# stevewongv/Sparse2Dense

Hardware: AMD Instinct MI355X
Metric: LiDAR frames/sec (fwd+bwd), 150k-pt 0.1m-voxel synthetic Waymo scene (higher is better)
Workload: dtype bf16 (sparse stack: bf16 storage; dense neck/head: bf16 NHWC activations; fp32 accumulate, statistics, master weights, optimizer)

## Files before the change

### include/s2d_debug.h

```cpp
#ifndef S2D_DEBUG_H
#define S2D_DEBUG_H

#include "s2d.h"

#ifdef __cplusplus
extern "C" {
#endif

int s2d_debug_lds_fill(float value, int blocks, int spin, float *sink, s2d_stream_t stream);

void s2d_debug_rg_trace(void *buf);

int s2d_conv2d_debug_force(int bm, int ns, int shared_a, int conv1x1_k64);

int s2d_conv2d_plan(int kind, int n, int h, int w, int cin, int cout, int pad, int stride, int ks, int32_t out[8]);

int s2d_conv2d_wgrad_debug_force(int ring_deep, int splits);

int s2d_conv2d_wgrad_plan(int kind, int n, int h, int w, int c_in_role, int c_out_role, int pad, int ks, int32_t out[8]);

#ifdef __cplusplus
}
#endif

#endif
```

### sparse2dense_amd/_lib.py

```python
import ctypes
import os

_HERE = os.path.dirname(os.path.abspath(__file__))
LIB_PATH = os.path.join(_HERE, "lib", "libs2d_hip.so")

c_i32p = ctypes.c_void_p
c_f32p = ctypes.c_void_p
_I3 = ctypes.c_int32 * 3
_PFN_GEO = [ctypes.c_int64, ctypes.c_int, ctypes.c_int, ctypes.c_float, ctypes.c_float, ctypes.c_float, ctypes.c_float]
_F3 = ctypes.c_float * 3
_F6 = ctypes.c_float * 6


class CenterTask(ctypes.Structure):
    _fields_ = [(n, ctypes.c_void_p) for n in ("hm_logit", "reg", "height", "dim", "vel", "rot", "hm", "ind", "mask", "cat", "anno_box", "p",
                                               "d_logit", "d_reg", "d_height", "d_dim", "d_vel", "d_rot")] + [("classes", ctypes.c_int)]

class CenterPredictTask(ctypes.Structure):
    _fields_ = [("map", ctypes.c_void_p * 6), ("channel_stride", ctypes.c_int64 * 6), ("pixel_stride", ctypes.c_int64 * 6),
                ("classes", ctypes.c_int), ("label_base", ctypes.c_int)]


class AnchorPredictTask(ctypes.Structure):
    _fields_ = [(n, ctypes.c_void_p) for n in ("box_preds", "cls_preds", "dir_cls_preds", "anchors")] + \
# ... 233 lines not shown
    "s2d_bev_iou_f32": (ctypes.c_int, [c_f32p, ctypes.c_int, c_f32p, ctypes.c_int, c_f32p, ctypes.c_void_p]),
    "s2d_nms_workspace_bytes": (ctypes.c_size_t, [ctypes.c_int]),
    "s2d_nms_rotated_bev": (ctypes.c_int, [c_f32p, ctypes.c_int, ctypes.c_float, ctypes.c_int, ctypes.c_void_p, ctypes.c_void_p, ctypes.c_void_p,
                                           ctypes.c_size_t, ctypes.c_void_p]),
    "s2d_nms_circle": (ctypes.c_int, [c_f32p, ctypes.c_int, ctypes.c_float, ctypes.c_int, ctypes.c_void_p, ctypes.c_void_p, ctypes.c_void_p,
                                      ctypes.c_size_t, ctypes.c_void_p]),
    "s2d_center_predict_score": (ctypes.c_int, [ctypes.c_void_p] + [ctypes.c_int] * 5 + [ctypes.c_float, ctypes.c_void_p] + [ctypes.c_float] * 5 +
                                 [ctypes.c_void_p] * 4),
    "s2d_center_predict_boxes": (ctypes.c_int, [ctypes.c_void_p] + [ctypes.c_int] * 5 + [ctypes.c_float] * 5 + [ctypes.c_void_p] * 5 +
                                 [ctypes.c_int, ctypes.c_int64] + [ctypes.c_void_p] * 4),
    "s2d_nms_batched_workspace_bytes": (ctypes.c_size_t, [ctypes.c_int64, ctypes.c_int]),
    "s2d_nms_rotated_bev_batched": (ctypes.c_int, [c_f32p, ctypes.c_int, c_i32p, c_i32p, ctypes.c_int, ctypes.c_int, ctypes.c_int64, ctypes.c_float,
                                                   ctypes.c_int, ctypes.c_void_p, ctypes.c_void_p, ctypes.c_void_p, ctypes.c_size_t, ctypes.c_void_p]),
    "s2d_nms_circle_batched": (ctypes.c_int, [c_f32p, ctypes.c_int, c_i32p, c_i32p, ctypes.c_int, ctypes.c_int, ctypes.c_int64, c_f32p,
                                              ctypes.c_int, ctypes.c_void_p, ctypes.c_void_p, ctypes.c_void_p, ctypes.c_size_t, ctypes.c_void_p]),
    "s2d_segment_topk": (ctypes.c_int, [ctypes.c_void_p, ctypes.c_int, ctypes.c_int64, ctypes.c_int64, ctypes.c_int, ctypes.c_void_p, ctypes.c_void_p,
                                        ctypes.c_void_p, ctypes.c_int64] + [ctypes.c_void_p] * 4),
    "s2d_predict_static_gather": (ctypes.c_int, [ctypes.c_void_p] * 6 + [ctypes.c_int] * 4 + [ctypes.c_int64] + [ctypes.c_void_p] * 5),
    "s2d_assign_label": (ctypes.c_int, [c_f32p, c_i32p, ctypes.c_int, ctypes.c_int, ctypes.c_float * 2, ctypes.c_float * 2] + [ctypes.c_int] * 5 +
                         [ctypes.c_double, ctypes.c_int] + [ctypes.c_void_p] * 7),
    "s2d_assign_label_tasks": (ctypes.c_int, [c_f32p, c_i32p, ctypes.c_int, ctypes.c_int, ctypes.POINTER(ctypes.c_int32), ctypes.c_int,
                                              ctypes.c_float * 2, ctypes.c_float * 2] + [ctypes.c_int] * 4 + [ctypes.c_double, ctypes.c_int] +
                               [ctypes.c_void_p] * 7),
    "s2d_adam_max_tensors": (ctypes.c_int, []),
    "s2d_adam_step_f32": (ctypes.c_int, [ctypes.c_int] + [ctypes.c_void_p] * 5 + [ctypes.c_float] * 5 + [ctypes.c_int, c_f32p, ctypes.c_void_p]),
    "s2d_grad_norm_workspace_floats": (ctypes.c_size_t, [ctypes.c_int, ctypes.c_void_p]),
    "s2d_grad_sumsq_f32": (ctypes.c_int, [ctypes.c_int, ctypes.c_void_p, ctypes.c_void_p, c_f32p, ctypes.c_void_p, ctypes.c_void_p]),
    "s2d_grad_norm_finalize_f32": (ctypes.c_int, [c_f32p, ctypes.c_int, ctypes.c_float, c_f32p, ctypes.c_void_p]),
    "s2d_dwconv7_supported": (ctypes.c_int, [ctypes.c_int]),
    "s2d_dwconv7_nhwc_bf16": (ctypes.c_int, [ctypes.c_void_p, c_f32p, c_f32p] + [ctypes.c_int] * 5 + [ctypes.c_void_p, ctypes.c_void_p]),
    "s2d_dwconv7_wgrad_workspace_bytes": (ctypes.c_size_t, [ctypes.c_int] * 4),
    "s2d_dwconv7_wgrad_nhwc_bf16": (ctypes.c_int, [ctypes.c_void_p, ctypes.c_void_p] + [ctypes.c_int] * 4 +
                                    [c_f32p, c_f32p, ctypes.c_void_p, ctypes.c_size_t, ctypes.c_void_p]),
    "s2d_comm_allreduce_sum_f32": (ctypes.c_int, [ctypes.c_void_p, ctypes.c_int64, ctypes.c_void_p]),
    "s2d_conv2d3x3_supported": (ctypes.c_int, [ctypes.c_int, ctypes.c_int]),
    "s2d_conv2d3x3_stats_tiles": (ctypes.c_int64, [ctypes.c_int] * 7),
    "s2d_conv2d3x3_pack_weights_bf16": (ctypes.c_int, [c_f32p, ctypes.c_int, ctypes.c_int, ctypes.c_int, ctypes.c_int,
                                                       ctypes.c_void_p, ctypes.c_void_p]),
    "s2d_conv2d3x3_tile_rows": (ctypes.c_int, [ctypes.c_int] * 7),
    "s2d_conv2d3x3_nhwc_bf16": (ctypes.c_int, [ctypes.c_void_p, ctypes.c_void_p, c_f32p, ctypes.c_void_p] +
                                [ctypes.c_int] * 7 + [ctypes.c_void_p, c_f32p, ctypes.c_void_p]),
    "s2d_bn_partials_finalize_f32": (ctypes.c_int, [c_f32p, ctypes.c_int, ctypes.c_int64, ctypes.c_int, c_f32p, c_f32p,
                                                    ctypes.c_float, ctypes.c_float, c_f32p, c_f32p, c_f32p, c_f32p, c_f32p, c_f32p,
                                                    ctypes.c_void_p, ctypes.c_void_p]),
    "s2d_bn_partials_finalize_ws_f32": (ctypes.c_int, [c_f32p, ctypes.c_int, ctypes.c_int64, ctypes.c_int, c_f32p, c_f32p,
                                                       ctypes.c_float, ctypes.c_float, c_f32p, c_f32p, c_f32p, c_f32p, c_f32p, c_f32p,
                                                       ctypes.c_void_p, ctypes.c_void_p, ctypes.c_size_t, ctypes.c_void_p]),
    "s2d_conv2d3x3_bnbwd_supported": (ctypes.c_int, [ctypes.c_int] * 4),
    "s2d_conv2d3x3_nhwc_bf16_bnbwd": (ctypes.c_int, [ctypes.c_void_p] * 3 + [ctypes.c_int] * 6 + [ctypes.c_void_p, ctypes.c_void_p, c_f32p, c_f32p,
                                                                                                    ctypes.c_int, c_f32p, ctypes.c_void_p]),
    "s2d_conv2d_debug_force": (ctypes.c_int, [ctypes.c_int] * 4),
    "s2d_conv2d_plan": (ctypes.c_int, [ctypes.c_int] * 9 + [ctypes.POINTER(ctypes.c_int32)]),
    "s2d_conv2d_wgrad_debug_force": (ctypes.c_int, [ctypes.c_int] * 2),
    "s2d_conv2d_wgrad_plan": (ctypes.c_int, [ctypes.c_int] * 8 + [ctypes.POINTER(ctypes.c_int32)]),
    "s2d_conv2d1x1_bnbwd_supported": (ctypes.c_int, [ctypes.c_int] * 2),
    "s2d_conv2d1x1_nhwc_bf16_bnbwd": (ctypes.c_int, [ctypes.c_void_p] * 3 + [ctypes.c_int] * 5 + [ctypes.c_void_p, ctypes.c_void_p, c_f32p, c_f32p,
                                                                                                    ctypes.c_int, c_f32p, ctypes.c_void_p]),
    "s2d_bn_partials_bwd_finalize_ws_f32": (ctypes.c_int, [c_f32p, ctypes.c_int, ctypes.c_int64, ctypes.c_int, c_f32p, c_f32p, c_f32p, c_f32p,
                                                           c_f32p, c_f32p, c_f32p, c_f32p, ctypes.c_void_p, ctypes.c_size_t, ctypes.c_void_p]),
    "s2d_bn_partials_sum_f32": (ctypes.c_int, [c_f32p, ctypes.c_int, ctypes.c_int64, ctypes.c_int, c_f32p, ctypes.c_int,
                                               ctypes.c_void_p]),
    "s2d_bn_partials_sum_workspace_bytes": (ctypes.c_size_t, [ctypes.c_int, ctypes.c_int]),
    "s2d_bn_partials_sum_ws_f32": (ctypes.c_int, [c_f32p, ctypes.c_int, ctypes.c_int64, ctypes.c_int, c_f32p, ctypes.c_int,
                                                  ctypes.c_void_p, ctypes.c_size_t, ctypes.c_void_p]),
    "s2d_bnrow_workspace_bytes": (ctypes.c_size_t, [ctypes.c_int64, ctypes.c_int]),
    "s2d_bnrow_stats_bf16": (ctypes.c_int, [ctypes.c_void_p, ctypes.c_int64, ctypes.c_int, c_f32p, ctypes.c_int, ctypes.c_void_p, ctypes.c_size_t, ctypes.c_void_p]),
    "s2d_bnrow_stats_finalize_bf16": (ctypes.c_int, [ctypes.c_void_p, ctypes.c_int64, ctypes.c_int, c_f32p, c_f32p, ctypes.c_float, ctypes.c_float, c_f32p, c_f32p, c_f32p, c_f32p, c_f32p, c_f32p, ctypes.c_void_p, ctypes.c_void_p, ctypes.c_size_t, ctypes.c_void_p]),
    "s2d_bnrow_apply_bf16": (ctypes.c_int, [ctypes.c_void_p, c_f32p, c_f32p, ctypes.c_void_p, ctypes.c_int, ctypes.c_int64, ctypes.c_int, ctypes.c_void_p, ctypes.c_void_p]),
    "s2d_bnrow_bwd_reduce_bf16": (ctypes.c_int, [ctypes.c_void_p, ctypes.c_void_p, ctypes.c_void_p, c_f32p, c_f32p, ctypes.c_int, ctypes.c_int64, ctypes.c_int, c_f32p, c_f32p, ctypes.c_void_p, ctypes.c_size_t, ctypes.c_void_p]),
    "s2d_bnrow_bwd_reduce_finalize_bf16": (ctypes.c_int, [ctypes.c_void_p, ctypes.c_void_p, ctypes.c_void_p, c_f32p, c_f32p, ctypes.c_int, ctypes.c_int64, ctypes.c_int, c_f32p, c_f32p, c_f32p, c_f32p, c_f32p, c_f32p, c_f32p, c_f32p, ctypes.c_void_p, ctypes.c_size_t, ctypes.c_void_p]),
    "s2d_bnrow_bwd_apply_bf16": (ctypes.c_int, [ctypes.c_void_p, ctypes.c_void_p, ctypes.c_void_p, c_f32p, c_f32p, ctypes.c_int, c_f32p, c_f32p, c_f32p, ctypes.c_int64, ctypes.c_int, ctypes.c_void_p, ctypes.c_void_p, ctypes.c_void_p]),
    "s2d_bnrow_apply_ld_bf16": (ctypes.c_int, [ctypes.c_void_p, c_f32p, c_f32p, ctypes.c_void_p, ctypes.c_int, ctypes.c_int64, ctypes.c_int, ctypes.c_void_p,
                                               ctypes.c_int, ctypes.c_void_p]),
    "s2d_bnrow_bwd_reduce_ld_bf16": (ctypes.c_int, [ctypes.c_void_p, ctypes.c_int, ctypes.c_void_p, ctypes.c_void_p, c_f32p, c_f32p, ctypes.c_int, ctypes.c_int64,
                                                    ctypes.c_int, c_f32p, c_f32p, ctypes.c_void_p, ctypes.c_size_t, ctypes.c_void_p]),
    "s2d_bnrow_bwd_reduce_finalize_ld_bf16": (ctypes.c_int, [ctypes.c_void_p, ctypes.c_int, ctypes.c_void_p, ctypes.c_void_p, c_f32p, c_f32p, ctypes.c_int,
                                                             ctypes.c_int64, ctypes.c_int, c_f32p, c_f32p, c_f32p, c_f32p, c_f32p, c_f32p, c_f32p, c_f32p,
                                                             ctypes.c_void_p, ctypes.c_size_t, ctypes.c_void_p]),
    "s2d_bnrow_bwd_apply_ld_bf16": (ctypes.c_int, [ctypes.c_void_p, ctypes.c_int, ctypes.c_void_p, ctypes.c_void_p, c_f32p, c_f32p, ctypes.c_int, c_f32p, c_f32p,
                                                   c_f32p, ctypes.c_int64, ctypes.c_int, ctypes.c_void_p, ctypes.c_void_p, ctypes.c_void_p]),
    "s2d_upsample2x_nhwc_bf16": (ctypes.c_int, [ctypes.c_void_p] + [ctypes.c_int] * 4 + [ctypes.c_void_p, ctypes.c_void_p]),
    "s2d_upsample2x_bwd_nhwc_bf16": (ctypes.c_int, [ctypes.c_void_p] + [ctypes.c_int] * 4 + [ctypes.c_void_p, ctypes.c_void_p]),
    "s2d_maxpool2x2_nhwc_bf16": (ctypes.c_int, [ctypes.c_void_p] + [ctypes.c_int] * 4 + [ctypes.c_void_p, ctypes.c_void_p]),
    "s2d_maxpool2x2_bwd_nhwc_bf16": (ctypes.c_int, [ctypes.c_void_p, ctypes.c_void_p] + [ctypes.c_int] * 4 + [ctypes.c_void_p, ctypes.c_void_p]),
    "s2d_spconv_s16_supported": (ctypes.c_int, [ctypes.c_int, ctypes.c_int]),
    "s2d_debug_rg_trace": (None, [ctypes.c_void_p]),
    "s2d_spconv_s16_packed_elems": (ctypes.c_size_t, [ctypes.c_int, ctypes.c_int, ctypes.c_int]),
    "s2d_spconv_s16_pack_weights": (ctypes.c_int, [c_f32p, ctypes.c_int, ctypes.c_int, ctypes.c_int, ctypes.c_int, ctypes.c_int,
                                                   ctypes.c_int64, ctypes.c_void_p, ctypes.c_void_p]),
    "s2d_spconv_s16_pack_weights_pair": (ctypes.c_int, [c_f32p, ctypes.c_int, ctypes.c_int, ctypes.c_int, ctypes.c_int, ctypes.c_int64,
                                                        ctypes.c_int64, ctypes.c_void_p, ctypes.c_void_p, ctypes.c_void_p]),
    "s2d_spconv_s16_fwd": (ctypes.c_int, [ctypes.c_void_p, ctypes.c_int64, ctypes.c_void_p, c_f32p, c_i32p, ctypes.c_int64,
                                          ctypes.c_int, ctypes.c_int, ctypes.c_int, ctypes.c_void_p, ctypes.c_void_p,
                                          ctypes.c_void_p]),
    "s2d_spconv_s16_stats_tiles": (ctypes.c_int64, [ctypes.c_int64, ctypes.c_int, ctypes.c_int, ctypes.c_int]),
    "s2d_spconv_s16_fwd_stats": (ctypes.c_int, [ctypes.c_void_p, ctypes.c_int64, ctypes.c_void_p, c_f32p, c_i32p, ctypes.c_int64,
                                                ctypes.c_int, ctypes.c_int, ctypes.c_int, ctypes.c_void_p, ctypes.c_void_p, c_f32p,
                                                ctypes.c_void_p]),
    "s2d_rulebook_sort_workspace_bytes": (ctypes.c_size_t, [ctypes.c_int64]),
    "s2d_rulebook_sort_chunk_rows": (ctypes.c_int64, [ctypes.c_int64]),
    "s2d_rulebook_sort_by_mask": (ctypes.c_int, [c_i32p, ctypes.c_int, ctypes.c_int64, c_i32p, ctypes.c_void_p, c_i32p, ctypes.c_void_p, ctypes.c_size_t,
                                                 ctypes.c_void_p]),
    "s2d_spconv_s16_set_sorted_rows": (ctypes.c_int, [ctypes.c_int]),
    "s2d_spconv_s16_sorted_supported": (ctypes.c_int, [ctypes.c_int] * 3),
    "s2d_spconv_s16_fwd_sorted": (ctypes.c_int, [ctypes.c_void_p, ctypes.c_int64, ctypes.c_void_p, c_f32p, c_i32p, c_i32p, ctypes.c_void_p, ctypes.c_int64,
                                                 ctypes.c_int, ctypes.c_int, ctypes.c_int, ctypes.c_void_p, c_f32p, ctypes.c_void_p]),
# ... 208 lines not shown
```

### sparse2dense_amd/csrc/convt3d_mfma.hip

```cpp
#include "s2d_common.h"
#include <algorithm>
#include <cstdlib>

namespace s2d {

typedef float f32x4m __attribute__((ext_vector_type(4)));
typedef __bf16 bf16x8m __attribute__((ext_vector_type(8)));

constexpr unsigned CT_OOB = BUF_OOB;
__device__ __forceinline__ __amdgpu_buffer_rsrc_t ct_rsrc(const void *base, unsigned bytes) { return buf_rsrc(base, bytes); }
__device__ __forceinline__ f32x4m ct_load4(__amdgpu_buffer_rsrc_t r, unsigned voff, unsigned soff) { return buf_load4(r, voff, soff); }
typedef uint32_t u32x2m __attribute__((ext_vector_type(2)));
typedef uint32_t u32x3m __attribute__((ext_vector_type(3)));
typedef uint32_t u32x4m __attribute__((ext_vector_type(4)));
__device__ __forceinline__ u32x3m ct_load3u(__amdgpu_buffer_rsrc_t r, unsigned voff, unsigned soff) {
    return __builtin_bit_cast(u32x3m, __builtin_amdgcn_raw_buffer_load_b96(r, voff, soff, 0));
}
__device__ __forceinline__ u32x4m ct_load4u(__amdgpu_buffer_rsrc_t r, unsigned voff, unsigned soff) {
    return __builtin_bit_cast(u32x4m, __builtin_amdgcn_raw_buffer_load_b128(r, voff, soff, 0));
}
__device__ __forceinline__ u32x2m ct_load2u(__amdgpu_buffer_rsrc_t r, unsigned voff, unsigned soff) {
    return __builtin_bit_cast(u32x2m, __builtin_amdgcn_raw_buffer_load_b64(r, voff, soff, 0));
}
__device__ __forceinline__ uint32_t ct_hi_hi(uint32_t a, uint32_t b) { return __builtin_amdgcn_perm(b, a, 0x07060302u); }
// ... 833 lines not shown
                f32x4m v0[MT], v1[MT];
#pragma unroll
                for (int mt = 0; mt < MT; ++mt) {
                    v0[mt] = ct_load4(dr, (pos[mt] | pl0) >= CT_OOB ? CT_OOB : pos[mt] + pl0, soff);
                    v1[mt] = ct_load4(dr, (pos[mt] | pl1) >= CT_OOB ? CT_OOB : pos[mt] + pl1, soff);
                }
#pragma unroll
                for (int mt = 0; mt < MT; ++mt) {
                    bf16x8m a;
#pragma unroll
                    for (int e = 0; e < 4; ++e) {
                        float s0 = shifted[mt] ? (e ? v0[mt][e - (e ? 1 : 0)] : 0.f) : v0[mt][e];
                        float s1 = shifted[mt] ? (e ? v1[mt][e - (e ? 1 : 0)] : 0.f) : v1[mt][e];
                        if (e == 3) {
                            s0 = last[mt] ? 0.f : s0;
                            s1 = last[mt] ? 0.f : s1;
                        }
                        a[e] = (__bf16)s0;
                        a[4 + e] = (__bf16)s1;
                    }
#pragma unroll
                    for (int nt = 0; nt < NT; ++nt) acc[mt][nt] = __builtin_amdgcn_mfma_f32_16x16x32_bf16(a, bfr[nt], acc[mt][nt], 0, 0, 0);
                }
                }
            }
        }
        const __amdgpu_buffer_rsrc_t ir = ct_rsrc(din + (int64_t)n * s.cin * cells, ibytes);
        const unsigned rowoff = (unsigned)(((int64_t)hz * s.h + hy) * s.w * IS);
#pragma unroll
        for (int mt = 0; mt < MT; ++mt) {
            const int c0 = x0 + mt * 16 + 4 * q;
#pragma unroll
            for (int nt = 0; nt < NT; ++nt) {
                const int ci = nt * 16 + r;
                const unsigned plane = ci < s.cin ? (unsigned)(ci * cells * IS) : CT_OOB;
                if constexpr (IS == 2) {
                    typedef __bf16 bf16x4i __attribute__((ext_vector_type(4)));
                    bf16x4i o;
#pragma unroll
                    for (int j = 0; j < 4; ++j) o[j] = (__bf16)acc[mt][nt][j];
                    buf_store2(ir, (c0 < s.w && ci < s.cin) ? plane + (unsigned)c0 * 2u : CT_OOB, rowoff, __builtin_bit_cast(buf_f32x2, o));
                } else if ((s.w & 3) == 0) {
                    buf_store4(ir, (c0 < s.w && ci < s.cin) ? plane + (unsigned)c0 * 4u : CT_OOB, rowoff, acc[mt][nt]);
                } else {
#pragma unroll
                    for (int j = 0; j < 4; ++j)
                        buf_store1(ir, (c0 + j < s.w && ci < s.cin) ? plane + (unsigned)(c0 + j) * 4u : CT_OOB, rowoff, acc[mt][nt][j]);
                }
            }
        }
    }
}

template <int CIT, int COT, int KG>
__global__ __launch_bounds__(256) void ct_wgrad_mfma_kernel(const float *__restrict__ x, const float *__restrict__ dout, CtDims s, int rows_per_block,
                                                            float *__restrict__ partial) {
    constexpr int FR = KG * 4 * CIT * COT;
    __shared__ float red[FR * 4][64];
    const int t = threadIdx.x, lane = t & 63, wid = t >> 6;
    const int r = lane & 15, q = lane >> 4;
    const int od = 2 * s.d, oh = 2 * s.h, ow = 2 * s.w;
    const int64_t cells = (int64_t)s.d * s.h * s.w, oplane = (int64_t)od * oh * ow;
    const int64_t total_rows = (int64_t)s.n * s.d * s.h;
    const int64_t r0 = (int64_t)blockIdx.x * rows_per_block;
    const int64_t r1 = r0 + rows_per_block < total_rows ? r0 + rows_per_block : total_rows;
    const int grp = blockIdx.y;
    f32x4m acc[KG][4][CIT][COT];
#pragma unroll
    for (int g = 0; g < KG; ++g)
#pragma unroll
        for (int k = 0; k < 4; ++k)
#pragma unroll
            for (int a = 0; a < CIT; ++a)
#pragma unroll
                for (int b = 0; b < COT; ++b) acc[g][k][a][b] = f32x4m{0.f, 0.f, 0.f, 0.f};
    const int steps = (s.w + 31) / 32;
    for (int64_t row = r0 + wid; row < r1; row += 4) {
        const int hy = (int)(row % s.h), hz = (int)((row / s.h) % s.d), n = (int)(row / ((int64_t)s.h * s.d));
        const float *xrow = x + (int64_t)n * s.cin * cells + ((int64_t)hz * s.h + hy) * s.w;
        const float *dbase = dout + (int64_t)n * s.cout * oplane;
        for (int st = 0; st < steps; ++st) {
            const int c0 = st * 32 + 8 * q;
            bf16x8m a[CIT];
#pragma unroll
            for (int ai = 0; ai < CIT; ++ai) {
                const int ci = ai * 16 + r;
#pragma unroll
                for (int e = 0; e < 8; ++e) a[ai][e] = (__bf16)0.f;
                if (ci < s.cin) {
                    const float *src = xrow + (int64_t)ci * cells + c0;
#pragma unroll
                    for (int e = 0; e < 8; ++e)
                        if (c0 + e < s.w) a[ai][e] = (__bf16)src[e];
                }
            }
#pragma unroll
            for (int g = 0; g < KG; ++g) {
                const int kzky = grp * KG + g;
                const int z = 2 * hz - 1 + (kzky >> 2), y = 2 * hy - 1 + (kzky & 3);
                if ((unsigned)z >= (unsigned)od || (unsigned)y >= (unsigned)oh) continue;
#pragma unroll
                for (int bi = 0; bi < COT; ++bi) {
                    const int co = bi * 16 + r;
                    float win[20];
#pragma unroll
                    for (int j = 0; j < 20; ++j) win[j] = 0.f;
// ... 460 lines not shown
        return S2D_OK;
    } else {
    if (ct_fwd_zslide(cin)) {
        const dim3 zgrid(xcd_grid((int64_t)batch * hg * xtiles)), zblk(256);
        if (nt == 2) hipLaunchKernelGGL((ct_fwd_zslide_kernel<16, 2, 4, TO>), zgrid, zblk, 0, st, in, wp, bias, s, xtiles, out, stats_partial, in_norm);
        else hipLaunchKernelGGL((ct_fwd_zslide_kernel<16, 1, 4, TO>), zgrid, zblk, 0, st, in, wp, bias, s, xtiles, out, stats_partial, in_norm);
        S2D_LAUNCH_CHECK();
        return S2D_OK;
    }
    const int64_t blocks = (int64_t)batch * d * hg * xtiles;
    S2D_CHECK_ARG(blocks < 0x7fffffff, "convt3d_mfma_fwd: grid too large");
    const dim3 grid(xcd_grid(blocks)), blk(256);
    const CtTileMap map = ct_tile_map(d, hg, xtiles, ct_chunk_rows((int64_t)w * cin * 4, yr, 2, 3));
    if (nt == 2) hipLaunchKernelGGL((ct_fwd_mfma_kernel<32, 2, 1, TO>), grid, blk, 0, st, in, wp, bias, s, xtiles, map, out, stats_partial, in_norm);
    else hipLaunchKernelGGL((ct_fwd_mfma_kernel<32, 1, 1, TO>), grid, blk, 0, st, in, wp, bias, s, xtiles, map, out, stats_partial, in_norm);
    S2D_LAUNCH_CHECK();
    return S2D_OK;
    }
}

extern "C" int s2d_convt3d_mfma_fwd_stats(const float *in, const void *packed, const float *bias, int batch, int cin, int cout, int d, int h,
                                          int w, float *out, float *stats_partial, s2d_stream_t stream) {
    return ct_fwd_launch<float>(in, packed, bias, batch, cin, cout, d, h, w, out, stats_partial, stream);
}
extern "C" int s2d_convt3d_mfma_fwd_stats_y16(const float *in, const void *packed, const float *bias, int batch, int cin, int cout, int d, int h,
                                              int w, void *out_bf16, float *stats_partial, s2d_stream_t stream) {
    return ct_fwd_launch<__bf16>(in, packed, bias, batch, cin, cout, d, h, w, (__bf16 *)out_bf16, stats_partial, stream);
}

extern "C" int s2d_convt3d_mfma_fwd_stats_y16_norm(const float *in, const float *in_scale_shift, const void *packed, const float *bias, int batch,
                                                   int cin, int cout, int d, int h, int w, void *out_bf16, float *stats_partial,
                                                   s2d_stream_t stream) {
    S2D_CHECK_ARG(in_scale_shift, "convt3d_mfma_fwd_stats_y16_norm: null scale / shift");
    if (!s2d_convt3d_mfma_norm_supported(cin, cout, d, h, w)) return S2D_ERR_UNSUPPORTED;
    return ct_fwd_launch<__bf16>(in, packed, bias, batch, cin, cout, d, h, w, (__bf16 *)out_bf16, stats_partial, stream, in_scale_shift);
}

extern "C" int s2d_convt3d_mfma_fwd_stats_y16_norm_x16(const void *in_bf16, const float *in_scale_shift, const void *packed, const float *bias,
                                                       int batch, int cin, int cout, int d, int h, int w, void *out_bf16, float *stats_partial,
                                                       s2d_stream_t stream) {
    S2D_CHECK_ARG(in_scale_shift, "convt3d_mfma_fwd_stats_y16_norm_x16: null scale / shift");
    if (!s2d_convt3d_mfma_x16_supported(cin, cout, d, h, w)) return S2D_ERR_UNSUPPORTED;
    return ct_fwd_launch<__bf16, __bf16>((const __bf16 *)in_bf16, packed, bias, batch, cin, cout, d, h, w, (__bf16 *)out_bf16, stats_partial, stream,
                                         in_scale_shift);
}

extern "C" int s2d_convt3d_mfma_fwd(const float *in, const void *packed, const float *bias, int batch, int cin, int cout, int d, int h,
                                    int w, float *out, s2d_stream_t stream) {
    return s2d_convt3d_mfma_fwd_stats(in, packed, bias, batch, cin, cout, d, h, w, out, nullptr, stream);
}

static bool ct_dgrad_is_direct(int cout, int d, int h, int w) { return (int64_t)cout * 8 * d * h * w * 4 < ((int64_t)1 << 31); }

template <typename TD, typename TI = float>
static int ct_dgrad_direct_launch(const TD *dout, const void *packed, int batch, int cin, int cout, int d, int h, int w, TI *din, hipStream_t st) {
    CtDims s{batch, d, h, w, cin, cout};
    const dim3 blk(256);
    const int nt_f = (cout + 15) / 16;
    const __bf16 *wp = (const __bf16 *)packed + (size_t)8 * (cin == 32 ? 8 : 4) * nt_f * 512;
    const bool narrow = cout <= 8;
    constexpr int MT = 4;
    const int tpr = (w + 16 * MT - 1) / (16 * MT);
    const int64_t items = (int64_t)batch * d * h * tpr;
    S2D_CHECK_ARG(items < 0x7fffffff, "convt3d_mfma_dgrad: too many tiles");
    const dim3 g2(xcd_grid(std::min<int64_t>(ceil_div(items, 4), 256 * 16)));
    const CtTileMap map = ct_tile_map(d, h, tpr, ct_chunk_rows((int64_t)2 * w * cout * sizeof(TD), 2, 2, 4));
    const __bf16 *wd = wp + (size_t)16 * (narrow ? 1 : 4) * (cin / 16) * 512;
    if constexpr (sizeof(TI) == 2) {
        if (!(narrow && cout <= 4 && cin == 16 && w % 4 == 0)) return S2D_ERR_UNSUPPORTED;
        hipLaunchKernelGGL((ct_dgrad_direct_kernel<8, 1, MT, true, TD, TI>), g2, blk, 0, st, dout, wd, s, tpr, map, din);
        S2D_LAUNCH_CHECK();
        return S2D_OK;
    } else
    if (narrow && cout <= 4 && cin == 32) hipLaunchKernelGGL((ct_dgrad_direct_kernel<8, 2, MT, true, TD>), g2, blk, 0, st, dout, wd, s, tpr, map, din);
    else if (narrow && cout <= 4) hipLaunchKernelGGL((ct_dgrad_direct_kernel<8, 1, MT, true, TD>), g2, blk, 0, st, dout, wd, s, tpr, map, din);
    else if (narrow && cin == 32) hipLaunchKernelGGL((ct_dgrad_direct_kernel<8, 2, MT, false, TD>), g2, blk, 0, st, dout, wd, s, tpr, map, din);
    else if (narrow) hipLaunchKernelGGL((ct_dgrad_direct_kernel<8, 1, MT, false, TD>), g2, blk, 0, st, dout, wd, s, tpr, map, din);
    else if (cin == 32) hipLaunchKernelGGL((ct_dgrad_direct_kernel<32, 2, MT, false, TD>), g2, blk, 0, st, dout, wd, s, tpr, map, din);
    else hipLaunchKernelGGL((ct_dgrad_direct_kernel<32, 1, MT, false, TD>), g2, blk, 0, st, dout, wd, s, tpr, map, din);
    S2D_LAUNCH_CHECK();
    return S2D_OK;
}

extern "C" int s2d_convt3d_mfma_dgrad(const float *dout, const void *packed, int batch, int cin, int cout, int d, int h, int w,
                                      float *din, s2d_stream_t stream) {
    S2D_CHECK_ARG(dout && packed && din && batch > 0 && d > 0 && h > 0 && w > 0, "convt3d_mfma_dgrad: bad argument");
    if (!ct_mfma_ok(cin, cout)) return S2D_ERR_UNSUPPORTED;
    hipStream_t st = (hipStream_t)stream;
    if (ct_dgrad_is_direct(cout, d, h, w)) return ct_dgrad_direct_launch<float>(dout, packed, batch, cin, cout, d, h, w, din, st);
    CtDims s{batch, d, h, w, cin, cout};
    const int xtiles = (w + CT_TX - 1) / CT_TX;
    const int64_t blocks = (int64_t)batch * d * h * xtiles;
    S2D_CHECK_ARG(blocks < 0x7fffffff, "convt3d_mfma_dgrad: grid too large");
    const dim3 grid((unsigned)blocks), blk(256);
    const int nt_f = (cout + 15) / 16;
    const __bf16 *wp = (const __bf16 *)packed + (size_t)8 * (cin == 32 ? 8 : 4) * nt_f * 512;
    const bool narrow = cout <= 8;
    if (narrow && cin == 32) hipLaunchKernelGGL((ct_dgrad_mfma_kernel<8, 2, 16>), grid, blk, 0, st, dout, wp, s, xtiles, din);
    else if (narrow) hipLaunchKernelGGL((ct_dgrad_mfma_kernel<8, 1, 16>), grid, blk, 0, st, dout, wp, s, xtiles, din);
    else if (cin == 32) hipLaunchKernelGGL((ct_dgrad_mfma_kernel<32, 2, 2>), grid, blk, 0, st, dout, wp, s, xtiles, din);
    else hipLaunchKernelGGL((ct_dgrad_mfma_kernel<32, 1, 2>), grid, blk, 0, st, dout, wp, s, xtiles, din);
    S2D_LAUNCH_CHECK();
    return S2D_OK;
}

extern "C" size_t s2d_convt3d_mfma_wgrad_workspace_bytes(int batch, int cin, int cout, int d, int h, int w) {
    if (batch <= 0 || d <= 0 || h <= 0 || w <= 0 || !ct_mfma_ok(cin, cout)) return 0;
    return align_up((size_t)ct_wgrad_blocks_for((int64_t)batch * d * h, cout, w) * cin * cout * 64 * sizeof(float), 256);
}

static bool ct_wgrad_has_d16(int cout, int w) { return ct_wgrad_is_narrow(cout, w) || w % 4 == 0; }

template <typename TD, typename TXI = float>
static int ct_wgrad_launch(const TXI *in, const TD *dout, int batch, int cin, int cout, int d, int h, int w, float *dweight, void *ws, hipStream_t st,
                           const float *in_norm = nullptr) {
    CtDims s{batch, d, h, w, cin, cout};
    const int64_t rows = (int64_t)batch * d * h;
    const int bx = ct_wgrad_blocks_for(rows, cout, w);
    const int rpb = (int)ceil_div(rows, bx);
    float *partial = (float *)ws;
    const int cit = cin / 16, cot = (cout + 15) / 16;
    const bool narrow = ct_wgrad_is_narrow(cout, w);
    if (in_norm && !ct_wgrad_has_d16(cout, w)) return S2D_ERR_UNSUPPORTED;
    if constexpr (sizeof(TXI) == 2) {
        if (!(narrow && cit == 1)) return S2D_ERR_UNSUPPORTED;
        hipLaunchKernelGGL((ct_wgrad_narrow_kernel<1, TD, TXI>), dim3(xcd_grid(bx)), dim3(256), 0, st, in, dout, s, rpb, bx, partial, in_norm);
    } else
    if (narrow && cit == 1) hipLaunchKernelGGL((ct_wgrad_narrow_kernel<1, TD>), dim3(xcd_grid(bx)), dim3(256), 0, st, in, dout, s, rpb, bx, partial, in_norm);
    else if (narrow) hipLaunchKernelGGL((ct_wgrad_narrow_kernel<2, TD>), dim3(xcd_grid(bx)), dim3(256), 0, st, in, dout, s, rpb, bx, partial, in_norm);
    else if (w % 4 == 0 && cit == 2) hipLaunchKernelGGL((ct_wgrad_rows_kernel<2, TD>), dim3(xcd_grid((int64_t)bx * 4 * cot)), dim3(256), 0, st, in, dout, s, rpb, cot, 4 * cot, bx, partial, in_norm);
    else if (w % 4 == 0) hipLaunchKernelGGL((ct_wgrad_rows_kernel<1, TD>), dim3(xcd_grid((int64_t)bx * 4 * cot * cit)), dim3(256), 0, st, in, dout, s, rpb, cot, 4 * cot * cit, bx, partial, in_norm);
    else if constexpr (sizeof(TD) == 4) {
// ... 383 lines not shown
```

Before: 223.4.

## Add row-grouped convT3d dgrad kernel sharing dout loads across two output rows

Adds a new transposed-3D-conv dgrad kernel that computes RY=2 adjacent input rows per wave, so overlapping dout rows loaded for neighbouring outputs are reused rather than fetched again. A new group tile map handles chunked row scheduling. By default it is used only for the bf16-input (TI=2) path; the fp32 path keeps the old kernel. A debug hook can force either mode and the chunk size. The cost is more accumulator registers per wave (RY×MT×NT fragments) and possibly lower occupancy.

```diff
diff --git a/include/s2d_debug.h b/include/s2d_debug.h
--- a/include/s2d_debug.h
+++ b/include/s2d_debug.h
@@ -19,6 +19,8 @@
 
 int s2d_conv2d_wgrad_plan(int kind, int n, int h, int w, int c_in_role, int c_out_role, int pad, int ks, int32_t out[8]);
 
+int s2d_convt3d_dgrad_debug_force(int group_mode, int chunk_rows);
+
 #ifdef __cplusplus
 }
 #endif
diff --git a/sparse2dense_amd/_lib.py b/sparse2dense_amd/_lib.py
--- a/sparse2dense_amd/_lib.py
+++ b/sparse2dense_amd/_lib.py
@@ -309,6 +309,7 @@
     "s2d_conv2d_debug_force": (ctypes.c_int, [ctypes.c_int] * 4),
     "s2d_conv2d_plan": (ctypes.c_int, [ctypes.c_int] * 9 + [ctypes.POINTER(ctypes.c_int32)]),
     "s2d_conv2d_wgrad_debug_force": (ctypes.c_int, [ctypes.c_int] * 2),
+    "s2d_convt3d_dgrad_debug_force": (ctypes.c_int, [ctypes.c_int] * 2),
     "s2d_conv2d_wgrad_plan": (ctypes.c_int, [ctypes.c_int] * 8 + [ctypes.POINTER(ctypes.c_int32)]),
     "s2d_conv2d1x1_bnbwd_supported": (ctypes.c_int, [ctypes.c_int] * 2),
     "s2d_conv2d1x1_nhwc_bf16_bnbwd": (ctypes.c_int, [ctypes.c_void_p] * 3 + [ctypes.c_int] * 5 + [ctypes.c_void_p, ctypes.c_void_p, c_f32p, c_f32p,
diff --git a/sparse2dense_amd/csrc/convt3d_mfma.hip b/sparse2dense_amd/csrc/convt3d_mfma.hip
--- a/sparse2dense_amd/csrc/convt3d_mfma.hip
+++ b/sparse2dense_amd/csrc/convt3d_mfma.hip
@@ -909,6 +909,177 @@
     }
 }
 
+struct CtGroupMap {
+    FastDiv per_n, per_chunk, per_plane, per_row;
+    int yc, items;
+};
+template <int RY>
+static inline CtGroupMap ct_group_map(int n, int d, int h, int xt, int yc) {
+    const int full = h / yc, tail = h - full * yc;
+    const int gy = (yc + RY - 1) / RY, gt = (tail + RY - 1) / RY;
+    const int per_n = d * xt * (full * gy + gt);
+    return CtGroupMap{fastdiv_make((uint32_t)per_n), fastdiv_make((uint32_t)(d * gy * xt)), fastdiv_make((uint32_t)(gy * xt)), fastdiv_make((uint32_t)xt),
+                      yc, n * per_n};
+}
+
+template <int COP, int NT, int MT, int RY, bool N4 = false, typename TD = float, typename TI = float>
+__global__ __launch_bounds__(256) void ct_dgrad_group_kernel(const TD *__restrict__ dout, const __bf16 *__restrict__ wp, CtDims s, int tiles_per_row,
+                                                             CtGroupMap map, TI *__restrict__ din) {
+    constexpr bool D16 = sizeof(TD) == 2;
+    constexpr unsigned ES = sizeof(TD);
+    constexpr unsigned IS = sizeof(TI);
+    constexpr int KSTEPS = COP == 32 ? 4 : 1;
+    constexpr int YSTEPS = N4 ? RY + 1 : 2 * RY + 2;
+    constexpr int YK = N4 ? 2 : 4, YSH = N4 ? 1 : 2;
+    const int lane = threadIdx.x & 63, wid = threadIdx.x >> 6;
+    const int r = lane & 15, q = lane >> 4;
+    const int od = 2 * s.d, oh = 2 * s.h, ow = 2 * s.w;
+    const int64_t cells = (int64_t)s.d * s.h * s.w, oplane = (int64_t)od * oh * ow;
+    const unsigned oplane_b = (unsigned)(oplane * ES), dbytes = (unsigned)(s.cout * oplane * ES), ibytes = (unsigned)(s.cin * cells * IS);
+    const int items = map.items;
+    const int xcd = blockIdx.x % S2D_XCDS, bx = blockIdx.x / S2D_XCDS, bpx = gridDim.x / S2D_XCDS;
+    const int per_xcd = (items + S2D_XCDS - 1) / S2D_XCDS;
+    const int it_hi = min(items, (xcd + 1) * per_xcd);
+    constexpr bool WREG = N4 && NT == 1 && KSTEPS == 1;
+    constexpr int ZU = WREG ? 4 : 1;
+    bf16x8m wreg[WREG ? 8 : 1];
+    if constexpr (WREG) {
+#pragma unroll
+        for (int k8 = 0; k8 < 8; ++k8) wreg[k8] = *reinterpret_cast<const bf16x8m *>(wp + ((int64_t)k8 * 64 + lane) * 8);
+    }
+    for (int item = xcd * per_xcd + bx * 4 + wid; item < it_hi; item += bpx * 4) {
+        const int n = (int)fastdiv((uint32_t)item, map.per_n);
+        int rem = item - n * (int)map.per_n.d;
+        const int chunk = (int)fastdiv((uint32_t)rem, map.per_chunk);
+        rem -= chunk * (int)map.per_chunk.d;
+        const int yc = min(map.yc, s.h - chunk * map.yc);
+        const int gy = (yc + RY - 1) / RY;
+        const int hz = yc == map.yc ? (int)fastdiv((uint32_t)rem, map.per_plane) : rem / (gy * tiles_per_row);
+        rem -= hz * (gy * tiles_per_row);
+        const int yg = (int)fastdiv((uint32_t)rem, map.per_row);
+        const int xt = rem - yg * tiles_per_row;
+        const int hy0 = chunk * map.yc + yg * RY;
+        const int nvy = min(RY, yc - yg * RY);
+        const __amdgpu_buffer_rsrc_t dr = ct_rsrc(dout + (int64_t)n * s.cout * oplane, dbytes);
+        const int x0 = xt * 16 * MT;
+        f32x4m acc[RY][MT][NT];
+        unsigned pos[MT];
+        bool shifted[MT], last[MT];
+#pragma unroll
+        for (int mt = 0; mt < MT; ++mt) {
+#pragma unroll
+            for (int iy = 0; iy < RY; ++iy)
+#pragma unroll
+                for (int nt = 0; nt < NT; ++nt) acc[iy][mt][nt] = f32x4m{0.f, 0.f, 0.f, 0.f};
+            const int c = x0 + mt * 16 + r;
+            shifted[mt] = c == 0;
+            last[mt] = c == s.w - 1;
+            pos[mt] = c < s.w ? (D16 ? (unsigned)((c == 0 ? 0 : 2 * c - 2) * 2) : (unsigned)((2 * c - (c == 0 ? 0 : 1)) * 4)) : CT_OOB;
+        }
+#pragma unroll ZU
+        for (int kz = 0; kz < 4; ++kz) {
+            const int z = 2 * hz - 1 + kz;
+#pragma unroll
+            for (int ys = 0; ys < YSTEPS; ++ys) {
+                const bool need = ys < YSH * nvy + YK - YSH;
+                const int y = 2 * hy0 - 1 + (N4 ? 2 * ys + (q >> 1) : ys);
+                const bool rok = need && (unsigned)z < (unsigned)od && (unsigned)y < (unsigned)oh;
+                const unsigned roff = rok ? (unsigned)(((int64_t)z * oh + y) * ow * ES) : 0u;
+                const unsigned soff = N4 ? 0u : roff;
+#pragma unroll
+                for (int ks = 0; ks < KSTEPS; ++ks) {
+                    const int co0 = N4 ? 2 * (q & 1) : 8 * ks + 2 * q;
+                    const unsigned pl0 = (rok && co0 < s.cout) ? (unsigned)co0 * oplane_b + (N4 ? roff : 0u) : CT_OOB;
+                    const unsigned pl1 = (rok && co0 + 1 < s.cout) ? (unsigned)(co0 + 1) * oplane_b + (N4 ? roff : 0u) : CT_OOB;
+                    bf16x8m a[MT];
+                    if constexpr (D16) {
+                        u32x3m u0[MT], u1[MT];
+#pragma unroll
+                        for (int mt = 0; mt < MT; ++mt) {
+                            u0[mt] = ct_load3u(dr, (pos[mt] | pl0) >= CT_OOB ? CT_OOB : pos[mt] + pl0, soff);
+                            u1[mt] = ct_load3u(dr, (pos[mt] | pl1) >= CT_OOB ? CT_OOB : pos[mt] + pl1, soff);
+                        }
+#pragma unroll
+                        for (int mt = 0; mt < MT; ++mt) {
+                            const bool sh = shifted[mt];
+                            const uint32_t a0 = sh ? 0u : u0[mt].x, a1 = sh ? u0[mt].x : u0[mt].y, a2 = sh ? u0[mt].y : u0[mt].z;
+                            const uint32_t b0 = sh ? 0u : u1[mt].x, b1 = sh ? u1[mt].x : u1[mt].y, b2 = sh ? u1[mt].y : u1[mt].z;
+                            const uint32_t lm = last[mt] ? 0x0000FFFFu : 0xFFFFFFFFu;
+                            const u32x4m pk = {__builtin_amdgcn_alignbit(a1, a0, 16), __builtin_amdgcn_alignbit(a2, a1, 16) & lm,
+                                               __builtin_amdgcn_alignbit(b1, b0, 16), __builtin_amdgcn_alignbit(b2, b1, 16) & lm};
+                            a[mt] = __builtin_bit_cast(bf16x8m, pk);
+                        }
+                    } else {
+                        f32x4m v0[MT], v1[MT];
+#pragma unroll
+                        for (int mt = 0; mt < MT; ++mt) {
+                            v0[mt] = ct_load4(dr, (pos[mt] | pl0) >= CT_OOB ? CT_OOB : pos[mt] + pl0, soff);
+                            v1[mt] = ct_load4(dr, (pos[mt] | pl1) >= CT_OOB ? CT_OOB : pos[mt] + pl1, soff);
+                        }
+#pragma unroll
+                        for (int mt = 0; mt < MT; ++mt) {
+#pragma unroll
+                            for (int e = 0; e < 4; ++e) {
+                                float s0 = shifted[mt] ? (e ? v0[mt][e - (e ? 1 : 0)] : 0.f) : v0[mt][e];
+                                float s1 = shifted[mt] ? (e ? v1[mt][e - (e ? 1 : 0)] : 0.f) : v1[mt][e];
+                                if (e == 3) {
+                                    s0 = last[mt] ? 0.f : s0;
+                                    s1 = last[mt] ? 0.f : s1;
+                                }
+                                a[mt][e] = (__bf16)s0;
+                                a[mt][4 + e] = (__bf16)s1;
+                            }
+                        }
+                    }
+#pragma unroll
+                    for (int iy = 0; iy < RY; ++iy) {
+                        const int kq = ys - YSH * iy;
+                        if (kq < 0 || kq >= YK) continue;
+                        const int entry = kz * YK + kq;
+#pragma unroll
+                        for (int nt = 0; nt < NT; ++nt) {
+                            bf16x8m b;
+                            if constexpr (WREG) b = wreg[entry];
+                            else b = *reinterpret_cast<const bf16x8m *>(wp + ((((int64_t)entry * KSTEPS + ks) * NT + nt) * 64 + lane) * 8);
+#pragma unroll
+                            for (int mt = 0; mt < MT; ++mt) acc[iy][mt][nt] = __builtin_amdgcn_mfma_f32_16x16x32_bf16(a[mt], b, acc[iy][mt][nt], 0, 0, 0);
+                        }
+                    }
+                }
+            }
+        }
+        const __amdgpu_buffer_rsrc_t ir = ct_rsrc(din + (int64_t)n * s.cin * cells, ibytes);
+#pragma unroll
+        for (int iy = 0; iy < RY; ++iy) {
+            if (iy >= nvy) continue;
+            const unsigned rowoff = (unsigned)(((int64_t)hz * s.h + hy0 + iy) * s.w * IS);
+#pragma unroll
+            for (int mt = 0; mt < MT; ++mt) {
+                const int c0 = x0 + mt * 16 + 4 * q;
+#pragma unroll
+                for (int nt = 0; nt < NT; ++nt) {
+                    const int ci = nt * 16 + r;
+                    const unsigned plane = ci < s.cin ? (unsigned)(ci * cells * IS) : CT_OOB;
+                    const f32x4m v = acc[iy][mt][nt];
+                    if constexpr (IS == 2) {
+                        typedef __bf16 bf16x4i __attribute__((ext_vector_type(4)));
+                        bf16x4i o;
+#pragma unroll
+                        for (int j = 0; j < 4; ++j) o[j] = (__bf16)v[j];
+                        buf_store2(ir, (c0 < s.w && ci < s.cin) ? plane + (unsigned)c0 * 2u : CT_OOB, rowoff, __builtin_bit_cast(buf_f32x2, o));
+                    } else if ((s.w & 3) == 0) {
+                        buf_store4(ir, (c0 < s.w && ci < s.cin) ? plane + (unsigned)c0 * 4u : CT_OOB, rowoff, v);
+                    } else {
+#pragma unroll
+                        for (int j = 0; j < 4; ++j)
+                            buf_store1(ir, (c0 + j < s.w && ci < s.cin) ? plane + (unsigned)(c0 + j) * 4u : CT_OOB, rowoff, v[j]);
+                    }
+                }
+            }
+        }
+    }
+}
+
 template <int CIT, int COT, int KG>
 __global__ __launch_bounds__(256) void ct_wgrad_mfma_kernel(const float *__restrict__ x, const float *__restrict__ dout, CtDims s, int rows_per_block,
                                                             float *__restrict__ partial) {
@@ -1475,32 +1646,68 @@
 
 static bool ct_dgrad_is_direct(int cout, int d, int h, int w) { return (int64_t)cout * 8 * d * h * w * 4 < ((int64_t)1 << 31); }
 
+static int g_ct_dgrad_mode = -1;
+static int g_ct_dgrad_chunk = -1;
+
+extern "C" int s2d_convt3d_dgrad_debug_force(int group_mode, int chunk_rows) {
+    S2D_CHECK_ARG(group_mode >= -1 && group_mode <= 1 && (chunk_rows == -1 || chunk_rows >= 1),
+                  "convt3d_dgrad_debug_force: group_mode -1/0/1, chunk_rows -1 or >= 1");
+    g_ct_dgrad_mode = group_mode;
+    g_ct_dgrad_chunk = chunk_rows;
+    return S2D_OK;
+}
+
+struct CtDgradArgs {
+    const void *dout, *wd;
+    void *din;
+    CtDims s;
+    hipStream_t st;
+};
+
+template <int COP, int NT, bool N4, typename TD, typename TI>
+static int ct_dgrad_direct_mode(const CtDgradArgs &a, int mode) {
+    const CtDims &s = a.s;
+    const dim3 blk(256);
+    const TD *dout = (const TD *)a.dout;
+    const __bf16 *wd = (const __bf16 *)a.wd;
+    TI *din = (TI *)a.din;
+    constexpr int MT = 4, RY = 2;
+    const int tpr = (s.w + 16 * MT - 1) / (16 * MT);
+    const int64_t items = (int64_t)s.n * s.d * s.h * tpr;
+    S2D_CHECK_ARG(items < 0x7fffffff, "convt3d_mfma_dgrad: too many tiles");
+    const int yc = g_ct_dgrad_chunk >= 1 ? g_ct_dgrad_chunk : ct_chunk_rows((int64_t)2 * s.w * s.cout * sizeof(TD), 2, 2, 4);
+    if (mode == 0) {
+        const dim3 g2(xcd_grid(std::min<int64_t>(ceil_div(items, 4), 256 * 16)));
+        const CtTileMap map = ct_tile_map(s.d, s.h, tpr, yc);
+        hipLaunchKernelGGL((ct_dgrad_direct_kernel<COP, NT, MT, N4, TD, TI>), g2, blk, 0, a.st, dout, wd, s, tpr, map, din);
+    } else {
+        const CtGroupMap map = ct_group_map<RY>(s.n, s.d, s.h, tpr, std::min(yc, s.h));
+        const dim3 g2(xcd_grid(std::min<int64_t>(ceil_div((int64_t)map.items, 4), 256 * 16)));
+        hipLaunchKernelGGL((ct_dgrad_group_kernel<COP, NT, MT, RY, N4, TD, TI>), g2, blk, 0, a.st, dout, wd, s, tpr, map, din);
+    }
+    return S2D_OK;
+}
+
 template <typename TD, typename TI = float>
 static int ct_dgrad_direct_launch(const TD *dout, const void *packed, int batch, int cin, int cout, int d, int h, int w, TI *din, hipStream_t st) {
-    CtDims s{batch, d, h, w, cin, cout};
-    const dim3 blk(256);
     const int nt_f = (cout + 15) / 16;
     const __bf16 *wp = (const __bf16 *)packed + (size_t)8 * (cin == 32 ? 8 : 4) * nt_f * 512;
     const bool narrow = cout <= 8;
-    constexpr int MT = 4;
-    const int tpr = (w + 16 * MT - 1) / (16 * MT);
-    const int64_t items = (int64_t)batch * d * h * tpr;
-    S2D_CHECK_ARG(items < 0x7fffffff, "convt3d_mfma_dgrad: too many tiles");
-    const dim3 g2(xcd_grid(std::min<int64_t>(ceil_div(items, 4), 256 * 16)));
-    const CtTileMap map = ct_tile_map(d, h, tpr, ct_chunk_rows((int64_t)2 * w * cout * sizeof(TD), 2, 2, 4));
     const __bf16 *wd = wp + (size_t)16 * (narrow ? 1 : 4) * (cin / 16) * 512;
+    const CtDgradArgs a{dout, wd, din, CtDims{batch, d, h, w, cin, cout}, st};
+    const int mode = g_ct_dgrad_mode >= 0 ? g_ct_dgrad_mode : (sizeof(TI) == 2 ? 1 : 0);
+    int rc;
     if constexpr (sizeof(TI) == 2) {
         if (!(narrow && cout <= 4 && cin == 16 && w % 4 == 0)) return S2D_ERR_UNSUPPORTED;
-        hipLaunchKernelGGL((ct_dgrad_direct_kernel<8, 1, MT, true, TD, TI>), g2, blk, 0, st, dout, wd, s, tpr, map, din);
-        S2D_LAUNCH_CHECK();
-        return S2D_OK;
+        rc = ct_dgrad_direct_mode<8, 1, true, TD, TI>(a, mode);
     } else
-    if (narrow && cout <= 4 && cin == 32) hipLaunchKernelGGL((ct_dgrad_direct_kernel<8, 2, MT, true, TD>), g2, blk, 0, st, dout, wd, s, tpr, map, din);
-    else if (narrow && cout <= 4) hipLaunchKernelGGL((ct_dgrad_direct_kernel<8, 1, MT, true, TD>), g2, blk, 0, st, dout, wd, s, tpr, map, din);
-    else if (narrow && cin == 32) hipLaunchKernelGGL((ct_dgrad_direct_kernel<8, 2, MT, false, TD>), g2, blk, 0, st, dout, wd, s, tpr, map, din);
-    else if (narrow) hipLaunchKernelGGL((ct_dgrad_direct_kernel<8, 1, MT, false, TD>), g2, blk, 0, st, dout, wd, s, tpr, map, din);
-    else if (cin == 32) hipLaunchKernelGGL((ct_dgrad_direct_kernel<32, 2, MT, false, TD>), g2, blk, 0, st, dout, wd, s, tpr, map, din);
-    else hipLaunchKernelGGL((ct_dgrad_direct_kernel<32, 1, MT, false, TD>), g2, blk, 0, st, dout, wd, s, tpr, map, din);
+    if (narrow && cout <= 4 && cin == 32) rc = ct_dgrad_direct_mode<8, 2, true, TD, TI>(a, mode);
+    else if (narrow && cout <= 4) rc = ct_dgrad_direct_mode<8, 1, true, TD, TI>(a, mode);
+    else if (narrow && cin == 32) rc = ct_dgrad_direct_mode<8, 2, false, TD, TI>(a, mode);
+    else if (narrow) rc = ct_dgrad_direct_mode<8, 1, false, TD, TI>(a, mode);
+    else if (cin == 32) rc = ct_dgrad_direct_mode<32, 2, false, TD, TI>(a, mode);
+    else rc = ct_dgrad_direct_mode<32, 1, false, TD, TI>(a, mode);
+    if (rc != S2D_OK) return rc;
     S2D_LAUNCH_CHECK();
     return S2D_OK;
 }
```

Measured after the change: 224.0, median of 3. About the same (+0.3%).
